# scart97/thunder-speech

Hardware: AMD Instinct MI355X
Metric: audio-seconds/s (16 kHz) QuartzNet15x5 inference (higher is better)
Workload: dtype bf16; 1 GPU; QuartzNet15x5 inference, batch 64x15 s per GPU, 16 kHz synthetic clips (BASELINE.json configs[1]); step = mel front end + 78 fused TCS launches + decoder + greedy decode (argmax + collapse), hipGraph replay; input_batches_rotated=5, input_bytes_rotated=307200000, batch_per_gpu=64, random_init=True, weights=random

## Files before the change

thunder_speech_amd/csrc/frontend.hip:

```cpp
#include "ts_common.hpp"
#include "ts_philox.hpp"

#include <cstdlib>

namespace ts {

constexpr int FPW = 16;
constexpr int NFFT = 512;
constexpr int NC = NFFT / 2;
constexpr float LOG_FLOOR = 5.9604644775390625e-08f;

struct Cx { float r, i; };
using C2 = f32x2;
__device__ __forceinline__ C2 cmul(C2 a, C2 w) { return C2{a[0], a[0]} * w + C2{a[1], a[1]} * C2{-w[1], w[0]}; }
__device__ __forceinline__ C2 mul_mi(C2 a) { return C2{a[1], -a[0]}; }
__device__ __forceinline__ C2 mul_pi(C2 a) { return C2{-a[1], a[0]}; }

__device__ __forceinline__ void fft16(C2 (&a)[16]) {
  C2 b[16];
#pragma unroll
  for (int n2 = 0; n2 < 4; ++n2) {
    const C2 s02 = a[n2] + a[8 + n2], d02 = a[n2] - a[8 + n2];
    const C2 s13 = a[4 + n2] + a[12 + n2], d13 = a[4 + n2] - a[12 + n2];
    b[n2 * 4 + 0] = s02 + s13;
    b[n2 * 4 + 1] = d02 + mul_mi(d13);
    b[n2 * 4 + 2] = s02 - s13;
    b[n2 * 4 + 3] = d02 + mul_pi(d13);
  }
  constexpr float C1 = 0.92387953251128674f, S1 = 0.38268343236508977f, R2 = 0.70710678118654752f;
  const C2 w[10] = {C2{1.f, 0.f}, C2{C1, -S1}, C2{R2, -R2}, C2{S1, -C1}, C2{0.f, -1.f},
                    C2{-S1, -C1}, C2{-R2, -R2}, C2{-C1, -S1}, C2{-1.f, 0.f}, C2{-C1, S1}};
#pragma unroll
  for (int n2 = 1; n2 < 4; ++n2)
#pragma unroll
    for (int k1 = 1; k1 < 4; ++k1) b[n2 * 4 + k1] = cmul(b[n2 * 4 + k1], w[n2 * k1]);
#pragma unroll
  for (int k1 = 0; k1 < 4; ++k1) {
    const C2 s02 = b[k1] + b[8 + k1], d02 = b[k1] - b[8 + k1];
    const C2 s13 = b[4 + k1] + b[12 + k1], d13 = b[4 + k1] - b[12 + k1];
    a[k1 + 0] = s02 + s13;
    a[k1 + 4] = d02 + mul_mi(d13);
    a[k1 + 8] = s02 - s13;
    a[k1 + 12] = d02 + mul_pi(d13);
  }
}

__device__ __forceinline__ void frame_sync() { asm volatile("s_waitcnt lgkmcnt(0)" ::: "memory"); }

struct FeArgs {
  const float* wave;
  const int* wave_len;
  const float* window;
  const float* mel_w;
  const int* mel_off;
  float* logmel;
  float* partial;
  int* feat_len;
  long long* feat_len64;
  int n_samples, hop, n_mels, n_frames, nwg, mel_nnz, batch;
  float preemph;
  float dither;
  unsigned long long seed;
};

__device__ __forceinline__ float dither_noise(unsigned long long seed, int b, int k) {
  const Philox4 r = philox(seed, PHILOX_DITHER, ((unsigned long long)(unsigned)b << 32) | (unsigned)(k >> 1));
  float n0, n1;
  normal2(r.v[0], r.v[1], n0, n1);
  return (k & 1) ? n1 : n0;
}

template <bool DITHER>
__global__ __launch_bounds__(256) void stft_mel_kernel(const FeArgs a) {
  extern __shared__ __attribute__((aligned(16))) char smem[];
  const int span = (FPW - 1) * a.hop + NFFT;
  float* const sig = reinterpret_cast<float*>(smem);
  Cx* const tw256 = reinterpret_cast<Cx*>(sig + round_up(span, 4));
  float* const win = reinterpret_cast<float*>(tw256 + NC);
  float* const fr = win + NFFT;
  constexpr int YSZ = 16 * 17 * 2;
  constexpr int FSZ = YSZ;
  static_assert(NC * 2 <= YSZ, "the spectrum of a frame fits the transpose tile it replaces");
  constexpr int RED0 = 288;
  float* const melw = fr + FPW * FSZ;
  int* const melo = reinterpret_cast<int*>(melw + a.mel_nnz);

  const int tid = threadIdx.x;
  const int T = a.n_samples;

  for (int j = tid; j < NC; j += 256) {
    float s, c;
    sincospif(-2.0f * (float)j / (float)NC, &s, &c);
    tw256[j] = Cx{c, s};
  }
  for (int j = tid; j < NFFT; j += 256) win[j] = a.window[j];
  for (int j = tid; j < a.mel_nnz; j += 256) melw[j] = a.mel_w[j];
  for (int j = tid; j < (a.n_mels + 1) * 2; j += 256) melo[j] = a.mel_off[j];

  constexpr int NV = 3;
  const int span4 = round_up(span, 4) / 4;
  const bool vec_ok = span4 <= 256 * NV && (T & 3) == 0 && ((FPW * a.hop) & 3) == 0 && (reinterpret_cast<uintptr_t>(a.wave) & 15) == 0;
  auto interior = [&](int g) {
    const int k0 = (g % a.nwg) * FPW * a.hop - NFFT / 2;
    return vec_ok && k0 >= 4 && k0 + 4 * span4 <= T;
  };
  f32x4 cur[NV];
  float prv[NV];
  auto fetch = [&](int g) {
    const float* x = a.wave + (size_t)(g / a.nwg) * a.n_samples + ((g % a.nwg) * FPW * a.hop - NFFT / 2);
#pragma unroll
    for (int j = 0; j < NV; ++j) {
      const int e = tid + 256 * j < span4 ? tid + 256 * j : span4 - 1;
      const float* const src = x + 4 * e;
      asm volatile("global_load_dwordx4 %0, %1, off" : "=v"(cur[j]) : "v"(src) : "memory");
      asm volatile("global_load_dword %0, %1, off offset:-4" : "=v"(prv[j]) : "v"(src) : "memory");
    }
  };
  auto commit = [&](int g) {
    static_assert(NV == 3, "operand list of the wait below");
    asm volatile("s_waitcnt vmcnt(0)" : "+v"(cur[0]), "+v"(cur[1]), "+v"(cur[2]), "+v"(prv[0]), "+v"(prv[1]), "+v"(prv[2]) :: "memory");
#pragma unroll
    for (int j = 0; j < NV; ++j) {
      const int e = tid + 256 * j;
      if constexpr (DITHER) {
        const int b = g / a.nwg, k = (g % a.nwg) * FPW * a.hop - NFFT / 2 + 4 * (e < span4 ? e : span4 - 1);
#pragma unroll
        for (int q = 0; q < 4; ++q) cur[j][q] += a.dither * dither_noise(a.seed, b, k + q);
        prv[j] += a.dither * dither_noise(a.seed, b, k - 1);
      }
      if (e < span4)
        *reinterpret_cast<f32x4*>(sig + 4 * e) = f32x4{cur[j][0] - a.preemph * prv[j], cur[j][1] - a.preemph * cur[j][0],
                                                       cur[j][2] - a.preemph * cur[j][1], cur[j][3] - a.preemph * cur[j][2]};
    }
  };
  auto stage_direct = [&](int g) {
    const float* x = a.wave + (size_t)(g / a.nwg) * a.n_samples;
    const int k0 = (g % a.nwg) * FPW * a.hop - NFFT / 2;
    for (int e = tid; e < span; e += 256) {
      int k = k0 + e;
      k = k < 0 ? -k : k;
      k = k >= T ? 2 * (T - 1) - k : k;
      k = k < 0 ? 0 : (k >= T ? T - 1 : k);
      float xc = x[k], xp = k > 0 ? x[k - 1] : 0.f;
      if constexpr (DITHER) {
        xc += a.dither * dither_noise(a.seed, g / a.nwg, k);
        if (k > 0) xp += a.dither * dither_noise(a.seed, g / a.nwg, k - 1);
      }
      sig[e] = xc - a.preemph * xp;
    }
  };
  const int n_groups = a.nwg * a.batch;
  int g = blockIdx.x;
  if (interior(g)) { fetch(g); commit(g); } else { stage_direct(g); }
  __syncthreads();

  for (; g < n_groups; g += gridDim.x) {
  const int b = g / a.nwg, grp = g - b * a.nwg;
  const int f0 = grp * FPW;
  const int gn = g + gridDim.x;
  const bool nvec = gn < n_groups && interior(gn);
  if (nvec) fetch(gn);

  const int fl = tid >> 4;
  const int i = tid & 15;
  float* const Y = fr + fl * FSZ;
  float* const Z = Y;
  {
    C2 v[16];
    const float* s = sig + fl * a.hop;
#pragma unroll
    for (int n1 = 0; n1 < 16; ++n1) {
      const int j = 32 * n1 + 2 * i;
      v[n1] = *reinterpret_cast<const f32x2*>(s + j) * *reinterpret_cast<const f32x2*>(win + j);
    }
    fft16(v);
#pragma unroll
    for (int k1 = 0; k1 < 16; ++k1)
      *reinterpret_cast<f32x2*>(Y + (k1 * 17 + i) * 2) = cmul(v[k1], *reinterpret_cast<const f32x2*>(&tw256[(i * k1) & (NC - 1)]));
  }
  frame_sync();
  {
    C2 v[16];
#pragma unroll
    for (int n2 = 0; n2 < 16; ++n2) v[n2] = *reinterpret_cast<const f32x2*>(Y + (i * 17 + n2) * 2);
    frame_sync();
    fft16(v);
#pragma unroll
    for (int k2 = 0; k2 < 16; ++k2) *reinterpret_cast<f32x2*>(Z + (i + 16 * k2) * 2) = v[k2];
  }
  frame_sync();
  float* const P = Y;
  {
    float pw[17];
    const f32x2 w_odd = (i & 1) ? f32x2{0.99992470183914454f, -0.012271538285719925f} : f32x2{1.f, 0.f};
#pragma unroll
    for (int j = 0; j < 17; ++j) {
      const int k = i + 16 * j;
      if (j < 16 || i == 0) {
        const f32x2 zk = *reinterpret_cast<const f32x2*>(Z + ((k & (NC - 1)) * 2));
        const f32x2 zn = *reinterpret_cast<const f32x2*>(Z + (((NC - k) & (NC - 1)) * 2));
        const f32x2 w = cmul(*reinterpret_cast<const f32x2*>(&tw256[(k >> 1) & (NC - 1)]), w_odd);
        const f32x2 znc = f32x2{zn[0], -zn[1]};
        const f32x2 A = zk + znc, D = zk - znc;
        const f32x2 wd = cmul(D, w);
        const f32x2 X = 0.5f * (A + f32x2{wd[1], -wd[0]});
        const float xr = X[0], xi = X[1];
        pw[j] = xr * xr + xi * xi;
      }
    }
    frame_sync();
#pragma unroll
    for (int j = 0; j < 17; ++j)
      if (j < 16 || i == 0) P[i + 16 * j] = pw[j];
  }
  frame_sync();
  const int f = f0 + fl;
  for (int m = i; m < a.n_mels; m += 16) {
    const int first = melo[2 * m], off = melo[2 * m + 1];
    const int cnt = melo[2 * m + 3] - off;
    float acc = 0.f;
    for (int j = 0; j < cnt; ++j) acc = fmaf(melw[off + j], P[first + j], acc);
    const float lm = logf(acc + LOG_FLOOR);
    fr[fl * FSZ + RED0 + m] = lm;
    if (f < a.n_frames) a.logmel[((size_t)b * a.n_frames + f) * a.n_mels + m] = lm;
  }
  __syncthreads();
  if (nvec) commit(gn);
  const int flen = a.wave_len[b] / a.hop + 1;
  if (tid == 0 && grp == 0) {
    a.feat_len[b] = flen;
    if (a.feat_len64) a.feat_len64[b] = flen;
  }
  for (int m = tid; m < a.n_mels; m += 256) {
    float s1 = 0.f, s2 = 0.f;
    for (int q = 0; q < FPW; ++q) {
      if (f0 + q < flen && f0 + q < a.n_frames) {
        const float v = fr[q * FSZ + RED0 + m];
        s1 += v;
        s2 = fmaf(v, v, s2);
      }
    }
    float* dst = a.partial + (((size_t)b * a.nwg + grp) * a.n_mels + m) * 2;
    dst[0] = s1;
    dst[1] = s2;
  }
  if (!nvec && gn < n_groups) stage_direct(gn);
  __syncthreads();
  }
}

struct NormArgs {
  const float* logmel;
  const float* partial;
  const int* feat_len;
  unsigned short* out;
  int n_mels, n_frames, nwg, pitch;
  const int* masks;
  int n_masks;
};

constexpr int NTF = 64;

__global__ __launch_bounds__(256) void normalize_kernel(const NormArgs a) {
  extern __shared__ __attribute__((aligned(16))) char smem[];
  float* const mean = reinterpret_cast<float*>(smem);
  float* const rstd = mean + a.n_mels;
  float* const tile = rstd + a.n_mels;
  const int tid = threadIdx.x;
  const int b = blockIdx.y;
  const int f0 = blockIdx.x * NTF;
  const int flen = a.feat_len[b] < a.n_frames ? a.feat_len[b] : a.n_frames;

  constexpr int NSL = 4;
  double* const slice = reinterpret_cast<double*>(tile);
  for (int idx = tid; idx < NSL * a.n_mels; idx += 256) {
    const int sl = idx / a.n_mels, m = idx - sl * a.n_mels;
    double s1 = 0.0, s2 = 0.0;
    const float* p = a.partial + ((size_t)b * a.nwg * a.n_mels + m) * 2;
    for (int w = sl; w < a.nwg; w += NSL) {
      s1 += (double)p[(size_t)w * a.n_mels * 2];
      s2 += (double)p[(size_t)w * a.n_mels * 2 + 1];
    }
    slice[idx * 2] = s1;
    slice[idx * 2 + 1] = s2;
  }
  __syncthreads();
  for (int m = tid; m < a.n_mels; m += 256) {
    double s1 = 0.0, s2 = 0.0;
    for (int sl = 0; sl < NSL; ++sl) {
      s1 += slice[(sl * a.n_mels + m) * 2];
      s2 += slice[(sl * a.n_mels + m) * 2 + 1];
    }
    const double n = (double)flen;
    const double mu = s1 / n;
    double var = (s2 - n * mu * mu + (double)(a.n_frames - flen) * mu * mu) / n;
    var = var < 0.0 ? 0.0 : var;
    mean[m] = (float)mu;
    rstd[m] = (float)(1.0 / (sqrt(var) + 1e-5));
  }
  __syncthreads();
  const int ld = a.n_mels + 1;
  for (int idx = tid; idx < NTF * a.n_mels; idx += 256) {
    const int q = idx / a.n_mels, m = idx - q * a.n_mels;
    const int f = f0 + q;
    tile[q * ld + m] = f < a.n_frames ? a.logmel[((size_t)b * a.n_frames + f) * a.n_mels + m] : 0.f;
  }
  __syncthreads();
  for (int idx = tid; idx < a.n_mels * (NTF / 8); idx += 256) {
    const int m = idx / (NTF / 8), g = idx - m * (NTF / 8);
    const float mu = mean[m], rs = rstd[m];
    float v[8];
#pragma unroll
    for (int j = 0; j < 8; ++j) {
      const int f = f0 + g * 8 + j;
      v[j] = f < flen ? (tile[(g * 8 + j) * ld + m] - mu) * rs : 0.f;
    }
    for (int r = 0; r < a.n_masks; ++r) {
      const int mf0 = a.masks[4 * r], mf1 = a.masks[4 * r + 1], mt0 = a.masks[4 * r + 2], mt1 = a.masks[4 * r + 3];
      if (m >= mf0 && m < mf1) {
#pragma unroll
        for (int j = 0; j < 8; ++j) {
          const int f = f0 + g * 8 + j;
          if (f >= mt0 && f < mt1) v[j] = 0.f;
        }
      }
    }
    if (f0 + g * 8 < a.pitch)
      *reinterpret_cast<u32x4*>(a.out + ((size_t)b * a.n_mels + m) * a.pitch + f0 + g * 8) =
          u32x4{pack_bf16(v[0], v[1]), pack_bf16(v[2], v[3]), pack_bf16(v[4], v[5]), pack_bf16(v[6], v[7])};
  }
}

static inline int fe_nwg(const ts_frontend_desc* d) { return (d->n_frames + FPW - 1) / FPW; }
static inline size_t fe_logmel_bytes(const ts_frontend_desc* d) {
  return round_up((size_t)d->batch * d->n_frames * d->n_mels * sizeof(float), 256);
}

}

extern "C" int64_t ts_frontend_workspace_bytes(const ts_frontend_desc* d) {
  if (!d || d->batch <= 0 || d->n_frames <= 0 || d->n_mels <= 0) return TS_EINVAL;
  return (int64_t)(ts::fe_logmel_bytes(d) + (size_t)d->batch * ts::fe_nwg(d) * d->n_mels * 2 * sizeof(float));
}

extern "C" const float* ts_frontend_logmel_ptr(const ts_frontend_desc* d, const void* workspace) {
  (void)d;
  return static_cast<const float*>(workspace);
}

namespace ts {
struct FeLaunch {
  int nwg, n_groups, grid, dither;
  size_t lds1;
};
}
static int fe_launch_config(const ts_frontend_desc* d, ts::FeLaunch* c) {
  using namespace ts;
  if (!d->window || !d->mel_weights || !d->mel_offsets) return TS_EINVAL;
  if (d->batch <= 0 || d->n_samples <= NFFT / 2 || d->hop <= 0 || d->n_mels <= 0) return TS_EINVAL;
  if (d->n_fft != NFFT) return TS_EUNSUPPORTED;
  if (d->win_length > NFFT || d->win_length <= 0) return TS_EINVAL;
  if (d->n_frames != d->n_samples / d->hop + 1) return TS_EINVAL;
  if (d->pitch_out % 8 || d->pitch_out < d->n_frames) return TS_EINVAL;
  if (d->n_masks < 0 || (d->n_masks > 0 && !d->masks)) return TS_EINVAL;
  if (d->mel_nnz < 0) return TS_EINVAL;
  if (d->n_mels > 256) return TS_EUNSUPPORTED;
  const long long span = (long long)(FPW - 1) * d->hop + NFFT;
  if (span > 160 * 1024 / 4) return TS_EUNSUPPORTED;
  const size_t lds1 = ((size_t)round_up((int)span, 4) + NC * 2 + NFFT + (size_t)FPW * (16 * 17 * 2) +
                       (size_t)d->mel_nnz + (size_t)(d->n_mels + 1) * 2) * sizeof(float);
  if (lds1 > 160 * 1024) return TS_EUNSUPPORTED;
  int per_cu = (int)((160 * 1024) / lds1) < 1 ? 1 : (int)((160 * 1024) / lds1);
  const int di = d->dither > 0.f ? 1 : 0;
  {
    static int occ_cache[64][2] = {};
    static size_t occ_lds[64][2] = {};
    int dev = 0;
    if (hipGetDevice(&dev) == hipSuccess && dev >= 0 && dev < 64) {
      if (occ_lds[dev][di] != lds1) {
        int occ = 0;
        const hipError_t oe = di ? hipOccupancyMaxActiveBlocksPerMultiprocessor(&occ, stft_mel_kernel<true>, 256, lds1)
                                 : hipOccupancyMaxActiveBlocksPerMultiprocessor(&occ, stft_mel_kernel<false>, 256, lds1);
        (void)hipGetLastError();
        occ_cache[dev][di] = (oe == hipSuccess && occ > 0) ? occ : per_cu;
        occ_lds[dev][di] = lds1;
      }
      if (occ_cache[dev][di] < per_cu) per_cu = occ_cache[dev][di];
    }
    (void)hipGetLastError();
  }
  c->nwg = fe_nwg(d);
  const long long n_groups = (long long)c->nwg * d->batch;
  if (n_groups > 2147483647LL) return TS_EINVAL;
  c->n_groups = (int)n_groups;
  c->grid = c->n_groups < cu_count() * per_cu ? c->n_groups : cu_count() * per_cu;
  c->dither = di;
  c->lds1 = lds1;
  return TS_OK;
}

extern "C" int ts_frontend_launch_config(const ts_frontend_desc* desc, int32_t* grid, int32_t* n_groups, int32_t* lds_bytes,
                                         int32_t* dither_instantiation) {
  if (!desc || !grid || !n_groups || !lds_bytes || !dither_instantiation) return TS_EINVAL;
  ts::FeLaunch c{};
  const int st = fe_launch_config(desc, &c);
  if (st != TS_OK) return st;
  *grid = c.grid; *n_groups = c.n_groups; *lds_bytes = (int32_t)c.lds1; *dither_instantiation = c.dither;
  return TS_OK;
}

extern "C" int ts_mel_frontend_fwd(const ts_frontend_desc* d, const float* wave, const int32_t* wave_len, void* features,
                                   int32_t* feat_len, void* workspace, void* stream_) {
  using namespace ts;
  if (!d || !wave || !wave_len || !features || !feat_len || !workspace) return TS_EINVAL;
  FeLaunch cfg{};
  const int cst = fe_launch_config(d, &cfg);
  if (cst != TS_OK) return cst;
  hipStream_t stream = reinterpret_cast<hipStream_t>(stream_);
  const int nwg = cfg.nwg;
  const size_t lds1 = cfg.lds1;

  FeArgs a{};
  a.wave = wave; a.wave_len = wave_len; a.window = d->window; a.mel_w = d->mel_weights; a.mel_off = d->mel_offsets;
  a.logmel = static_cast<float*>(workspace);
  a.partial = reinterpret_cast<float*>(static_cast<char*>(workspace) + fe_logmel_bytes(d));
  a.feat_len = feat_len;
  a.feat_len64 = reinterpret_cast<long long*>(d->feat_len64);
  a.n_samples = d->n_samples; a.hop = d->hop; a.n_mels = d->n_mels; a.n_frames = d->n_frames; a.nwg = nwg;
  a.preemph = d->preemph;
  a.dither = d->dither;
  a.seed = d->dither_seed;
  a.mel_nnz = d->mel_nnz;
  a.batch = d->batch;
  if (lds1 > 64 * 1024) {
    hipError_t e1 = hipFuncSetAttribute(reinterpret_cast<const void*>(stft_mel_kernel<false>), hipFuncAttributeMaxDynamicSharedMemorySize, (int)lds1);
    if (e1 == hipSuccess) e1 = hipFuncSetAttribute(reinterpret_cast<const void*>(stft_mel_kernel<true>), hipFuncAttributeMaxDynamicSharedMemorySize, (int)lds1);
    if (e1 != hipSuccess) return (int)e1;
  }
  const size_t lds2 = ((size_t)2 * d->n_mels + (size_t)NTF * (d->n_mels + 1)) * sizeof(float);
  if (lds2 > 64 * 1024) {
    const hipError_t e2 = hipFuncSetAttribute(reinterpret_cast<const void*>(normalize_kernel), hipFuncAttributeMaxDynamicSharedMemorySize, (int)lds2);
    if (e2 != hipSuccess) return (int)e2;
  }
  (void)hipGetLastError();
  if (cfg.dither) hipLaunchKernelGGL(stft_mel_kernel<true>, dim3(cfg.grid), dim3(256), lds1, stream, a);
  else hipLaunchKernelGGL(stft_mel_kernel<false>, dim3(cfg.grid), dim3(256), lds1, stream, a);
  hipError_t e = hipGetLastError();
  if (e != hipSuccess) return (int)e;

  NormArgs n{};
  n.logmel = a.logmel; n.partial = a.partial; n.feat_len = feat_len; n.out = static_cast<unsigned short*>(features);
  n.n_mels = d->n_mels; n.n_frames = d->n_frames; n.nwg = nwg; n.pitch = d->pitch_out;
  n.masks = d->masks; n.n_masks = d->n_masks;
  (void)hipGetLastError();
  hipLaunchKernelGGL(normalize_kernel, dim3((d->pitch_out + NTF - 1) / NTF, d->batch), dim3(256), lds2, stream, n);
  return hip_status(hipGetLastError());
}
```

Baseline: 321,800 audio-seconds/s.

## Shrink STFT LDS tile, use DPP for spectrum partners, vectorize normalize loads

The STFT/mel front end now moves the transpose through LDS as separate real and imaginary passes, which shrinks the per-frame tile. It keeps the second FFT's output in registers and fetches the mirrored bins with DPP row shuffles instead of an LDS round-trip. Launch bounds and the LDS budget are retuned so more workgroups fit per CU, with the per-CU count capped by a register-based limit. Smaller changes chunk the mel dot product, batch the partial-sum loads, and vectorize the logmel tile load in the normalize kernel. The front end is only a small share of the full step, so any end-to-end effect is likely small. The added instructions and explicit FP contraction and reassociation control keep results bit-exact, at the cost of extra code complexity.

```diff
diff --git a/thunder_speech_amd/csrc/frontend.hip b/thunder_speech_amd/csrc/frontend.hip
--- a/thunder_speech_amd/csrc/frontend.hip
+++ b/thunder_speech_amd/csrc/frontend.hip
@@ -9,6 +9,16 @@
 constexpr int NFFT = 512;
 constexpr int NC = NFFT / 2;
 constexpr float LOG_FLOOR = 5.9604644775390625e-08f;
+constexpr int FE_WAVES = 4;
+constexpr int FE_WAVES_DITHER = 3;
+constexpr int FE_MEL_CHUNK = 4;
+
+constexpr int FE_YSZ = 16 * 17;
+constexpr int FE_RED0 = 260;
+__host__ __device__ constexpr int fe_tile_floats(int n_mels) {
+  const int need = FE_RED0 + n_mels > FE_YSZ ? FE_RED0 + n_mels : FE_YSZ;
+  return (need + 15) / 32 * 32 + 16;
+}
 
 struct Cx { float r, i; };
 using C2 = f32x2;
@@ -46,6 +56,21 @@
 }
 
 __device__ __forceinline__ void frame_sync() { asm volatile("s_waitcnt lgkmcnt(0)" ::: "memory"); }
+__device__ __forceinline__ void frame_order() { asm volatile("" ::: "memory"); }
+
+__device__ __forceinline__ float square(float x) {
+#pragma clang fp contract(off)
+  return x * x;
+}
+__device__ __forceinline__ float power_two_products(float xr, float xi) {
+#pragma clang fp contract(off)
+  return xr * xr + xi * xi;
+}
+
+__device__ __forceinline__ float row_partner(float x, float own) {
+  const int m = __builtin_amdgcn_update_dpp(0, __float_as_int(x), 0x140, 0xf, 0xf, false);
+  return __int_as_float(__builtin_amdgcn_update_dpp(__float_as_int(own), m, 0x111, 0xf, 0xf, false));
+}
 
 struct FeArgs {
   const float* wave;
@@ -71,17 +96,16 @@
 }
 
 template <bool DITHER>
-__global__ __launch_bounds__(256) void stft_mel_kernel(const FeArgs a) {
+__global__ __launch_bounds__(256, DITHER ? FE_WAVES_DITHER : FE_WAVES) void stft_mel_kernel(const FeArgs a) {
   extern __shared__ __attribute__((aligned(16))) char smem[];
   const int span = (FPW - 1) * a.hop + NFFT;
   float* const sig = reinterpret_cast<float*>(smem);
   Cx* const tw256 = reinterpret_cast<Cx*>(sig + round_up(span, 4));
   float* const win = reinterpret_cast<float*>(tw256 + NC);
   float* const fr = win + NFFT;
-  constexpr int YSZ = 16 * 17 * 2;
-  constexpr int FSZ = YSZ;
-  static_assert(NC * 2 <= YSZ, "the spectrum of a frame fits the transpose tile it replaces");
-  constexpr int RED0 = 288;
+  const int FSZ = fe_tile_floats(a.n_mels);
+  constexpr int RED0 = FE_RED0;
+  static_assert(NC + 1 <= FE_RED0, "the power spectrum of a frame ends below its log-mel staging");
   float* const melw = fr + FPW * FSZ;
   int* const melo = reinterpret_cast<int*>(melw + a.mel_nnz);
 
@@ -164,54 +188,51 @@
   const int fl = tid >> 4;
   const int i = tid & 15;
   float* const Y = fr + fl * FSZ;
-  float* const Z = Y;
+  float* const P = Y;
   {
     C2 v[16];
-    const float* s = sig + fl * a.hop;
-#pragma unroll
-    for (int n1 = 0; n1 < 16; ++n1) {
-      const int j = 32 * n1 + 2 * i;
-      v[n1] = *reinterpret_cast<const f32x2*>(s + j) * *reinterpret_cast<const f32x2*>(win + j);
+    {
+      const float* s = sig + fl * a.hop;
+#pragma unroll
+      for (int n1 = 0; n1 < 16; ++n1) {
+        const int j = 32 * n1 + 2 * i;
+        v[n1] = *reinterpret_cast<const f32x2*>(s + j) * *reinterpret_cast<const f32x2*>(win + j);
+      }
+      fft16(v);
+#pragma unroll
+      for (int k1 = 0; k1 < 16; ++k1) v[k1] = cmul(v[k1], *reinterpret_cast<const f32x2*>(&tw256[(i * k1) & (NC - 1)]));
+      float re[16];
+#pragma unroll
+      for (int k1 = 0; k1 < 16; ++k1) Y[k1 * 17 + i] = v[k1][0];
+      frame_sync();
+#pragma unroll
+      for (int n2 = 0; n2 < 16; ++n2) re[n2] = Y[i * 17 + n2];
+      frame_order();
+#pragma unroll
+      for (int k1 = 0; k1 < 16; ++k1) Y[k1 * 17 + i] = v[k1][1];
+      frame_sync();
+#pragma unroll
+      for (int n2 = 0; n2 < 16; ++n2) v[n2] = C2{re[n2], Y[i * 17 + n2]};
+      frame_sync();
     }
     fft16(v);
-#pragma unroll
-    for (int k1 = 0; k1 < 16; ++k1)
-      *reinterpret_cast<f32x2*>(Y + (k1 * 17 + i) * 2) = cmul(v[k1], *reinterpret_cast<const f32x2*>(&tw256[(i * k1) & (NC - 1)]));
-  }
-  frame_sync();
-  {
-    C2 v[16];
-#pragma unroll
-    for (int n2 = 0; n2 < 16; ++n2) v[n2] = *reinterpret_cast<const f32x2*>(Y + (i * 17 + n2) * 2);
-    frame_sync();
-    fft16(v);
-#pragma unroll
-    for (int k2 = 0; k2 < 16; ++k2) *reinterpret_cast<f32x2*>(Z + (i + 16 * k2) * 2) = v[k2];
-  }
-  frame_sync();
-  float* const P = Y;
-  {
-    float pw[17];
     const f32x2 w_odd = (i & 1) ? f32x2{0.99992470183914454f, -0.012271538285719925f} : f32x2{1.f, 0.f};
 #pragma unroll
     for (int j = 0; j < 17; ++j) {
       const int k = i + 16 * j;
+      f32x2 zn = v[0];
+      if (j < 16) zn = f32x2{row_partner(v[15 - j][0], v[(16 - j) & 15][0]), row_partner(v[15 - j][1], v[(16 - j) & 15][1])};
       if (j < 16 || i == 0) {
-        const f32x2 zk = *reinterpret_cast<const f32x2*>(Z + ((k & (NC - 1)) * 2));
-        const f32x2 zn = *reinterpret_cast<const f32x2*>(Z + (((NC - k) & (NC - 1)) * 2));
+        const f32x2 zk = v[j & 15];
         const f32x2 w = cmul(*reinterpret_cast<const f32x2*>(&tw256[(k >> 1) & (NC - 1)]), w_odd);
         const f32x2 znc = f32x2{zn[0], -zn[1]};
         const f32x2 A = zk + znc, D = zk - znc;
         const f32x2 wd = cmul(D, w);
         const f32x2 X = 0.5f * (A + f32x2{wd[1], -wd[0]});
         const float xr = X[0], xi = X[1];
-        pw[j] = xr * xr + xi * xi;
-      }
-    }
-    frame_sync();
-#pragma unroll
-    for (int j = 0; j < 17; ++j)
-      if (j < 16 || i == 0) P[i + 16 * j] = pw[j];
+        P[k] = j == 14 || j == 15 ? power_two_products(xr, xi) : fmaf(xr, xr, square(xi));
+      }
+    }
   }
   frame_sync();
   const int f = f0 + fl;
@@ -219,7 +240,24 @@
     const int first = melo[2 * m], off = melo[2 * m + 1];
     const int cnt = melo[2 * m + 3] - off;
     float acc = 0.f;
-    for (int j = 0; j < cnt; ++j) acc = fmaf(melw[off + j], P[first + j], acc);
+    constexpr int MC = FE_MEL_CHUNK;
+    const float* const wr = melw + off;
+    const float* const pr = P + first;
+    int j0 = 0;
+    for (; j0 + MC <= cnt; j0 += MC) {
+      float w[MC], p[MC];
+#pragma unroll
+      for (int q = 0; q < MC; ++q) { w[q] = wr[j0 + q]; p[q] = pr[j0 + q]; }
+#pragma unroll
+      for (int q = 0; q < MC; ++q) acc = fmaf(w[q], p[q], acc);
+    }
+    if (j0 < cnt) {
+      float w[MC], p[MC];
+#pragma unroll
+      for (int q = 0; q < MC - 1; ++q) { w[q] = wr[j0 + q]; p[q] = pr[j0 + q]; }
+#pragma unroll
+      for (int q = 0; q < MC - 1; ++q) acc = j0 + q < cnt ? fmaf(w[q], p[q], acc) : acc;
+    }
     const float lm = logf(acc + LOG_FLOOR);
     fr[fl * FSZ + RED0 + m] = lm;
     if (f < a.n_frames) a.logmel[((size_t)b * a.n_frames + f) * a.n_mels + m] = lm;
@@ -233,11 +271,17 @@
   }
   for (int m = tid; m < a.n_mels; m += 256) {
     float s1 = 0.f, s2 = 0.f;
-    for (int q = 0; q < FPW; ++q) {
-      if (f0 + q < flen && f0 + q < a.n_frames) {
-        const float v = fr[q * FSZ + RED0 + m];
-        s1 += v;
-        s2 = fmaf(v, v, s2);
+    float lm[FPW];
+#pragma unroll
+    for (int q = 0; q < FPW; ++q) lm[q] = fr[q * FSZ + RED0 + m];
+    {
+#pragma clang fp reassociate(off)
+#pragma unroll
+      for (int q = 0; q < FPW; ++q) {
+        if (f0 + q < flen && f0 + q < a.n_frames) {
+          s1 += lm[q];
+          s2 = fmaf(lm[q], lm[q], s2);
+        }
       }
     }
     float* dst = a.partial + (((size_t)b * a.nwg + grp) * a.n_mels + m) * 2;
@@ -277,9 +321,25 @@
     const int sl = idx / a.n_mels, m = idx - sl * a.n_mels;
     double s1 = 0.0, s2 = 0.0;
     const float* p = a.partial + ((size_t)b * a.nwg * a.n_mels + m) * 2;
-    for (int w = sl; w < a.nwg; w += NSL) {
-      s1 += (double)p[(size_t)w * a.n_mels * 2];
-      s2 += (double)p[(size_t)w * a.n_mels * 2 + 1];
+    constexpr int NU = 8;
+    for (int w0 = sl; w0 < a.nwg; w0 += NSL * NU) {
+      float t1[NU], t2[NU];
+#pragma unroll
+      for (int u = 0; u < NU; ++u) {
+        const int w = w0 + NSL * u < a.nwg ? w0 + NSL * u : a.nwg - 1;
+        t1[u] = p[(size_t)w * a.n_mels * 2];
+        t2[u] = p[(size_t)w * a.n_mels * 2 + 1];
+      }
+      {
+#pragma clang fp reassociate(off)
+#pragma unroll
+        for (int u = 0; u < NU; ++u) {
+          if (w0 + NSL * u < a.nwg) {
+            s1 += (double)t1[u];
+            s2 += (double)t2[u];
+          }
+        }
+      }
     }
     slice[idx * 2] = s1;
     slice[idx * 2 + 1] = s2;
@@ -300,10 +360,38 @@
   }
   __syncthreads();
   const int ld = a.n_mels + 1;
-  for (int idx = tid; idx < NTF * a.n_mels; idx += 256) {
-    const int q = idx / a.n_mels, m = idx - q * a.n_mels;
-    const int f = f0 + q;
-    tile[q * ld + m] = f < a.n_frames ? a.logmel[((size_t)b * a.n_frames + f) * a.n_mels + m] : 0.f;
+  if ((a.n_mels & 3) == 0 && (reinterpret_cast<uintptr_t>(a.logmel) & 15) == 0) {
+    const int r4 = a.n_mels >> 2;
+    const int dq = 256 / r4, dc = 256 - dq * r4;
+    int q = tid / r4, c = tid - q * r4;
+    constexpr int NL = 4;
+    for (int idx = tid; idx < NTF * r4; idx += 256 * NL) {
+      f32x4 v[NL];
+      int qs[NL], cs[NL];
+#pragma unroll
+      for (int u = 0; u < NL; ++u) {
+        qs[u] = q; cs[u] = c;
+        const int f = f0 + q < a.n_frames ? f0 + q : a.n_frames - 1;
+        v[u] = *reinterpret_cast<const f32x4*>(a.logmel + ((size_t)b * a.n_frames + f) * a.n_mels + 4 * c);
+        q += dq; c += dc;
+        if (c >= r4) { c -= r4; ++q; }
+      }
+#pragma unroll
+      for (int u = 0; u < NL; ++u) {
+        if (idx + 256 * u < NTF * r4) {
+          const bool in = f0 + qs[u] < a.n_frames;
+          float* const t = tile + qs[u] * ld + 4 * cs[u];
+#pragma unroll
+          for (int e = 0; e < 4; ++e) t[e] = in ? v[u][e] : 0.f;
+        }
+      }
+    }
+  } else {
+    for (int idx = tid; idx < NTF * a.n_mels; idx += 256) {
+      const int q = idx / a.n_mels, m = idx - q * a.n_mels;
+      const int f = f0 + q;
+      tile[q * ld + m] = f < a.n_frames ? a.logmel[((size_t)b * a.n_frames + f) * a.n_mels + m] : 0.f;
+    }
   }
   __syncthreads();
   for (int idx = tid; idx < a.n_mels * (NTF / 8); idx += 256) {
@@ -367,11 +455,13 @@
   if (d->n_mels > 256) return TS_EUNSUPPORTED;
   const long long span = (long long)(FPW - 1) * d->hop + NFFT;
   if (span > 160 * 1024 / 4) return TS_EUNSUPPORTED;
-  const size_t lds1 = ((size_t)round_up((int)span, 4) + NC * 2 + NFFT + (size_t)FPW * (16 * 17 * 2) +
-                       (size_t)d->mel_nnz + (size_t)(d->n_mels + 1) * 2) * sizeof(float);
+  const size_t lds1 = ((size_t)round_up((int)span, 4) + NC * 2 + NFFT + (size_t)FPW * fe_tile_floats(d->n_mels) +
+                       (size_t)d->mel_nnz + (size_t)(d->n_mels + 1) * 2 + FE_MEL_CHUNK) * sizeof(float);
   if (lds1 > 160 * 1024) return TS_EUNSUPPORTED;
   int per_cu = (int)((160 * 1024) / lds1) < 1 ? 1 : (int)((160 * 1024) / lds1);
   const int di = d->dither > 0.f ? 1 : 0;
+  const int by_regs = di ? FE_WAVES_DITHER : FE_WAVES;
+  if (per_cu > by_regs) per_cu = by_regs;
   {
     static int occ_cache[64][2] = {};
     static size_t occ_lds[64][2] = {};
```

After: 324,300 audio-seconds/s (median of 6 runs). Within noise of the previous version (+0.8%).
